# bartn8/vppstereo

Hardware: AMD Instinct MI355X
Metric: Mdisparities/s (HxWxD / s) VPP+rSGM at 540x960xD=192 (higher is better)
Workload: dtype u16

## Files before the change

vppstereo_amd/csrc/rsgm_kernels.hip:

```cpp
#include "vppx_internal.h"

#include <stdlib.h>

#define INVALID_DISP_COST 16u
#define INVALID_DISP (-10.0f)

typedef u32 u32x4 __attribute__((ext_vector_type(4)));
typedef u32 u32x2 __attribute__((ext_vector_type(2)));
typedef u16 u16x2 __attribute__((ext_vector_type(2)));

__device__ __forceinline__ u32 pk_min(u32 a, u32 b)
{
    u16x2 r = __builtin_elementwise_min(__builtin_bit_cast(u16x2, a), __builtin_bit_cast(u16x2, b));
    return __builtin_bit_cast(u32, r);
}
__device__ __forceinline__ u32 pk_adds(u32 a, u32 b)
{
    u16x2 r = __builtin_elementwise_add_sat(__builtin_bit_cast(u16x2, a), __builtin_bit_cast(u16x2, b));
    return __builtin_bit_cast(u32, r);
}
__device__ __forceinline__ u32 pk_sub(u32 a, u32 b)
{
    u16x2 r = __builtin_bit_cast(u16x2, a) - __builtin_bit_cast(u16x2, b);
    return __builtin_bit_cast(u32, r);
// ... 3724 lines not shown
    }
    return __builtin_amdgcn_fmed3f(fmaxf(fmaxf(lo[0], lo[1]), lo[2]), __builtin_amdgcn_fmed3f(md[0], md[1], md[2]),
                                   fminf(fminf(hi[0], hi[1]), hi[2]));
}
__global__ void __launch_bounds__(256) median3x3_kernel(const float *__restrict__ src, float *__restrict__ dst, int Hp, int Wp)
{
    const int x = blockIdx.x * blockDim.x + threadIdx.x;
    const int y = blockIdx.y;
    const int f = blockIdx.z;
    if (x >= Wp) return;
    const float *s = src + (size_t)f * Hp * Wp;
    float out;
    if (y == 0 || y == Hp - 1 || x == 0 || x == Wp - 1) {
        out = s[(size_t)y * Wp + x];
    } else {
        float v[9];
#pragma unroll
        for (int dy = -1; dy <= 1; dy++)
#pragma unroll
            for (int dx = -1; dx <= 1; dx++) v[(dy + 1) * 3 + dx + 1] = s[(size_t)(y + dy) * Wp + x + dx];
        out = median9(v);
    }
    dst[((size_t)f * Hp + y) * Wp + x] = out;
}

int rsgm_launch_median(vppx_ctx *ctx, int B, int Hp, int Wp, const float *src, float *dst)
{
    dim3 grid((Wp + 255) / 256, Hp, B);
    median3x3_kernel<<<grid, 256, 0, ctx->stream>>>(src, dst, Hp, Wp);
    VPPX_CHECK_LAUNCH();
    return 0;
}

__global__ void __launch_bounds__(256) median_interp_clip_kernel(ImgSet io, int B, int Hp, int Wp)
{
    extern __shared__ __attribute__((aligned(16))) float s_med[];
    const int nwords = (Wp + 63) / 64;
    unsigned long long *s_bits = (unsigned long long *)(s_med + ((Wp + 1) & ~1));
    const int y = blockIdx.x;
    const int set = blockIdx.y / B, f = blockIdx.y % B;
    const int lane = threadIdx.x & 63;
    const float *s = (const float *)(set == 0 ? io.src[0] : io.src[1]) + (size_t)f * Hp * Wp;
    float *dst = (float *)(set == 0 ? io.dst[0] : io.dst[1]) + ((size_t)f * Hp + y) * Wp;
    if (threadIdx.x == 0) s_bits[0] = 0ull, s_bits[nwords + 1] = 0ull;
    for (int xb = threadIdx.x & ~63; xb < Wp; xb += 256) {
        const int x = xb + lane;
        float out = 0.0f;
        if (x < Wp) {
            if (y == 0 || y == Hp - 1 || x == 0 || x == Wp - 1) {
                out = s[(size_t)y * Wp + x];
            } else {
                float v[9];
#pragma unroll
                for (int dy = -1; dy <= 1; dy++)
#pragma unroll
                    for (int dx = -1; dx <= 1; dx++) v[(dy + 1) * 3 + dx + 1] = s[(size_t)(y + dy) * Wp + x + dx];
                out = median9(v);
            }
            s_med[x] = out;
        }
        const unsigned long long bal = __builtin_amdgcn_ballot_w64(x < Wp && out > 0);
        if (lane == 0) s_bits[1 + (xb >> 6)] = bal;
    }
    __syncthreads();
    const float *row = s_med;
    const u32 *b32 = (const u32 *)s_bits;
    for (int x = threadIdx.x; x < Wp; x += 256) {
        float v = row[x];
        if (v <= 0) {
            const int sb = 64 + x - 13;
            const u32 w = __builtin_amdgcn_alignbit(b32[(sb >> 5) + 1], b32[sb >> 5], (u32)(sb & 31)) & 0x7FFFFFFu;
            const u32 wl = w & 0x1FFFu;
            int xl = -1, xr = -1;
            if (wl) {
                xl = x - 13 + (31 - __builtin_clz(wl));
                const int top = 27 - (x - xl);
                const u32 wr = (w >> 14) & ((1u << (top - 13)) - 1u);
                if (wr) xr = x + 1 + __builtin_ctz(wr);
            }
            if (xl >= 0 && xr >= 0) {
                const double n_left = (double)row[xl], n_right = (double)row[xr];
                if (fabs(n_left - n_right) < 3.0) {
                    const int xt = max(xl + 1, xr - 7);
                    const int n_leftx = xl - xt, n_rightx = xr - xt;
                    const double m = __ddiv_rn(n_right - n_left, (double)(n_rightx - n_leftx));
                    const double q = __dsub_rn(n_left, __dmul_rn(m, (double)n_leftx));
                    v = (float)__dadd_rn(__dmul_rn(m, (double)(x - xt)), q);
                }
            }
        }
        dst[x] = (v >= 0) ? v : 0.0f;
    }
}

int rsgm_launch_median_interp_clip(vppx_ctx *ctx, int B, int Hp, int Wp, const float *src_l, float *dst_l, const float *src_r,
                                   float *dst_r)
{
    ImgSet io;
    io.src[0] = src_l; io.dst[0] = dst_l; io.src[1] = src_r; io.dst[1] = dst_r; io.src[2] = nullptr; io.dst[2] = nullptr;
    const size_t lds = (size_t)((Wp + 1) & ~1) * sizeof(float) + (size_t)((Wp + 63) / 64 + 3) * sizeof(unsigned long long);
    median_interp_clip_kernel<<<dim3(Hp, 2 * B), 256, lds, ctx->stream>>>(io, B, Hp, Wp);
    VPPX_CHECK_LAUNCH();
    return 0;
}

__device__ __forceinline__ int uf_find(int *label, int i)
{
    int p = label[i];
    while (p != i) {
        i = p;
        p = label[i];
    }
    return i;
}
__device__ __forceinline__ int uf_find_halve(int *label, int i)
{
    int p = label[i];
    while (p != i) {
        const int gp = label[p];
        if (gp != p) atomicMin(&label[i], gp);
        i = p;
        p = gp;
    }
    return i;
}
__device__ __forceinline__ void uf_union(int *label, int a, int b)
{
    while (true) {
        a = uf_find_halve(label, a);
        b = uf_find_halve(label, b);
        if (a == b) return;
        if (a < b) { int t = a; a = b; b = t; }
        const int old = atomicMin(&label[a], b);
        if (old == a) return;
// ... 173 lines not shown
    }
    uf_union(lb, lb[ia], lb[ib]);
}

__global__ void __launch_bounds__(64) speckle_total_kernel(int *__restrict__ label, int *__restrict__ size, const int *__restrict__ roots,
                                                           const int *__restrict__ nroots, size_t npix_frame, int tiles_per_frame)
{
    const int tile = blockIdx.x;
    const size_t base = (size_t)(tile / tiles_per_frame) * npix_frame;
    int *lb = label + base;
    const int n = nroots[tile];
    const int *rl = roots + (size_t)tile * (SPK_TW * SPK_TH);
    for (int e = threadIdx.x; e < n; e += 64) {
        const int me = rl[e];
        const int sz = size[base + me];
        int c = me, p = lb[c];
        while (p != c) {
            const int gp = lb[p];
            if (gp != p) lb[c] = gp;
            c = gp;
            p = lb[c];
        }
        if (c != me) {
            lb[me] = c;
            atomicAdd(&size[base + c], sz);
        }
    }
}

template <int SEGMAX>
__global__ void __launch_bounds__(256) speckle_apply_rows_kernel(const u8 *__restrict__ fd8, const int *__restrict__ label,
                                                                  const int *__restrict__ size, const float *__restrict__ dl_pad,
                                                                  float *__restrict__ out, u8 *__restrict__ row_any, int H, int W, int Hp,
                                                                  int Wp, int pad_t, int pad_l, int new_val, int max_size, int subpixel)
{
    extern __shared__ __attribute__((aligned(16))) float sh_f[];
    __shared__ int s_l[4], s_r[4];
    float *val = sh_f, *res = sh_f + W;
    const int y = blockIdx.x, f = blockIdx.y;
    const int lane = threadIdx.x & 63, wv = threadIdx.x >> 6;
    const size_t base = (size_t)f * H * W, rowo = base + (size_t)y * W;
    const int *lb = label + base;
    const float *dlr = dl_pad + ((size_t)f * Hp + y + pad_t) * Wp + pad_l;
    float *g = out + rowo;
    for (int xb = threadIdx.x; xb < W; xb += 4 * 256) {
        int v[4], r1[4], r2[4];
        float sub[4];
#pragma unroll
        for (int u = 0; u < 4; u++) {
            const int x = min(xb + 256 * u, W - 1);
            v[u] = fd8[rowo + x];
            r1[u] = label[rowo + x];
            sub[u] = dlr[x];
        }
#pragma unroll
        for (int u = 0; u < 4; u++) r2[u] = lb[r1[u]];
#pragma unroll
        for (int u = 0; u < 4; u++) {
            int r = r1[u], pr = r2[u];
            while (pr != r) {
                r = pr;
                pr = lb[r];
            }
            r1[u] = r;
        }
        int sz[4];
#pragma unroll
        for (int u = 0; u < 4; u++) sz[u] = size[base + r1[u]];
#pragma unroll
        for (int u = 0; u < 4; u++) {
            const int x = xb + 256 * u;
            int vv = v[u];
            if (vv != new_val && sz[u] <= max_size) vv = new_val;
            float fv = (float)vv;
            if (subpixel && fv != 0.0f) fv = sub[u];
            if (x < W) val[x] = fv;
        }
// ... 25 lines not shown
    if (lane == 63) cr = 0x7FFFFFFF;
    for (int w = 0; w < wv; w++) cl = max(cl, s_l[w]);
    for (int w = wv + 1; w < 4; w++) cr = min(cr, s_r[w]);
    int xl[SEGMAX];
#pragma unroll
    for (int j = 0; j < SEGMAX; j++) {
        const int x = x0 + j;
        if (j < SEG && x < W && val[x] > 0) cl = x;
        xl[j] = cl;
    }
#pragma unroll
    for (int j = SEGMAX - 1; j >= 0; j--) {
        const int x = x0 + j;
        if (j >= SEG || x >= W) continue;
        float v = val[x];
        if (v > 0) {
            cr = x;
        } else {
            const bool hl = xl[j] >= 0, hr = cr < W;
            if (hl && hr) {
                const float a = val[xl[j]], b = val[cr];
                v = b < a ? b : a;
            } else if (hr) {
                v = val[cr];
            } else if (hl) {
                v = val[xl[j]];
            }
        }
        res[x] = v;
    }
    __syncthreads();
    for (int x = threadIdx.x; x < W; x += 256) g[x] = res[x];
}
__global__ void __launch_bounds__(256) interp_bg_edge_rows_kernel(float *__restrict__ dm, const u8 *__restrict__ row_any, int H, int W)
{
    __shared__ int s_first[4], s_last[4];
    const int f = blockIdx.x, lane = threadIdx.x & 63, wv = threadIdx.x >> 6;
    float *g = dm + (size_t)f * H * W;
    int first = 0x7FFFFFFF, last = -1;
    for (int v = threadIdx.x; v < H; v += 256)
        if (row_any[(size_t)f * H + v]) { first = min(first, v); last = max(last, v); }
#pragma unroll
    for (int off = 32; off >= 1; off >>= 1) {
        first = min(first, __shfl_xor(first, off));
        last = max(last, __shfl_xor(last, off));
    }
    if (lane == 0) s_first[wv] = first, s_last[wv] = last;
    __syncthreads();
    first = min(min(s_first[0], s_first[1]), min(s_first[2], s_first[3]));
    last = max(max(s_last[0], s_last[1]), max(s_last[2], s_last[3]));
    if (last < 0) return;
    for (size_t i = threadIdx.x; i < (size_t)first * W; i += 256) g[i] = g[(size_t)first * W + i % W];
    for (size_t i = (size_t)(last + 1) * W + threadIdx.x; i < (size_t)H * W; i += 256) g[i] = g[(size_t)last * W + i % W];
}

__global__ void __launch_bounds__(256) void_if_lost_kernel(float *__restrict__ out, size_t n, const unsigned *__restrict__ err_dev,
                                                           unsigned serial)
{
    if (__hip_atomic_load(err_dev, __ATOMIC_RELAXED, __HIP_MEMORY_SCOPE_AGENT) != serial) return;
    const float nan = __builtin_nanf("");
    for (size_t i = (size_t)blockIdx.x * 256 + threadIdx.x; i < n; i += (size_t)gridDim.x * 256) out[i] = nan;
}

int rsgm_launch_void_if_lost(vppx_ctx *ctx, float *out, size_t n, const unsigned *err_dev, unsigned serial)
{
    const unsigned nblk = (unsigned)((n + 256 * 16 - 1) / (256 * 16));
    void_if_lost_kernel<<<nblk < 1 ? 1 : nblk, 256, 0, ctx->stream>>>(out, n, err_dev, serial);
    VPPX_CHECK_LAUNCH();
    return 0;
}

int rsgm_launch_post(vppx_ctx *ctx, const RsgmGeom &g, const float *dl_pad, const float *dr_pad, int subpixel, float *out)
{
    const size_t n = (size_t)g.B * g.H * g.W, npf = (size_t)g.H * g.W;
    if (g.W > 8192) { vppx_set_error("frame width %d > 8192 is not supported by the post-processing kernels", g.W); return VPPX_E_UNSUPPORTED; }
    const int ntx = (g.W + SPK_TW - 1) / SPK_TW, nty = (g.H + SPK_TH - 1) / SPK_TH;
    const size_t ntiles = (size_t)ntx * nty * g.B;
    u8 *fd8, *row_any;
    int *label, *size, *roots, *nroots;
    int rc;
    if ((rc = ws_get(ctx, WS_FD8, n, &fd8))) return rc;
    if ((rc = ws_get(ctx, WS_LABEL, n, &label))) return rc;
    if ((rc = ws_get(ctx, WS_LCOUNT, n, &size))) return rc;
    if ((rc = ws_get(ctx, WS_SPK_ROOTS, ntiles * (SPK_TW * SPK_TH), &roots))) return rc;
    if ((rc = ws_get(ctx, WS_SPK_NROOTS, ntiles, &nroots))) return rc;
    if ((rc = ws_get(ctx, WS_ROW_ANY, (size_t)g.B * g.H, &row_any))) return rc;
    speckle_tile_kernel<<<dim3(ntx, nty, g.B), 256, 0, ctx->stream>>>(dl_pad, dr_pad, fd8, label, size, roots, nroots, g.H, g.W, g.Hp, g.Wp,
                                                                      g.pad_t, g.pad_l, 0, 10);
    VPPX_CHECK_LAUNCH();
    const int nby = (g.H - 1) / SPK_TH, nbx = (g.W - 1) / SPK_TW;
    const int nlinks = nby * g.W + nbx * g.H;
    if (nlinks > 0) {
        speckle_border_kernel<<<dim3((nlinks + 255) / 256, g.B), 256, 0, ctx->stream>>>(fd8, label, g.H, g.W, 0, 10);
        VPPX_CHECK_LAUNCH();
    }
    speckle_total_kernel<<<(unsigned)ntiles, 64, 0, ctx->stream>>>(label, size, roots, nroots, npf, ntx * nty);
    VPPX_CHECK_LAUNCH();
    const size_t lds = (size_t)g.W * 2 * sizeof(float);
    if (g.W <= 2048)
        speckle_apply_rows_kernel<8><<<dim3(g.H, g.B), 256, lds, ctx->stream>>>(fd8, label, size, dl_pad, out, row_any, g.H, g.W, g.Hp, g.Wp,
                                                                               g.pad_t, g.pad_l, 0, 200, subpixel);
    else
        speckle_apply_rows_kernel<32><<<dim3(g.H, g.B), 256, lds, ctx->stream>>>(fd8, label, size, dl_pad, out, row_any, g.H, g.W, g.Hp, g.Wp,
                                                                                g.pad_t, g.pad_l, 0, 200, subpixel);
    VPPX_CHECK_LAUNCH();
    interp_bg_edge_rows_kernel<<<g.B, 256, 0, ctx->stream>>>(out, row_any, g.H, g.W);
    VPPX_CHECK_LAUNCH();
    return 0;
}
```

vppstereo_amd/csrc/vpp_kernels.hip:

```cpp
#include "vppx_internal.h"

#include <math.h>
#include <string.h>
#include <mutex>
#include <stdlib.h>

#define LG 992
#define RLCAP 8

struct HintRec {
    int x;
    float g;
    u32 base;
    u32 flags;
};

__host__ __device__ inline int vpp_bits_words(int W) { return (W + 63) / 64 + 2; }

struct VppK {
    int B, H, W, C;
    int n, direction, uniform, discard, interp, use_dist, use_bil;
    int wsize_m1;
    float c, c_occ, dmin, dmax;
    const float2 *range;
// ... 2028 lines not shown
    const int x = blockIdx.x * blockDim.x + threadIdx.x;
    const int y = blockIdx.y, f = blockIdx.z;
    if (x >= W) return;
    const size_t fb = (size_t)f * H * W;
    auto unwarped = [&](int yy, int xx) -> float {
        const size_t row = fb + (size_t)yy * W;
        const int t = tmp[row + xx];
        return t < 0 ? 0.0f : omap[row + (t >> 1)];
    };
    float u = unwarped(y, x);
    if (u == 0.0f) {
        const float nl = x > 0 ? unwarped(y, x - 1) : unwarped(y, W - 1);
        const float nr = x < W - 1 ? unwarped(y, x + 1) : (y < H - 1 ? unwarped(y + 1, 0) : 0.0f);
        if (nl > 0 && nr > 0 && fabs(__dsub_rn((double)nl, (double)nr)) < 1.0) {
            const double m = __ddiv_rn(__dsub_rn((double)nr, (double)nl), 2.0);
            const double q = __dsub_rn((double)nl, __dmul_rn(m, -1.0));
            u = (float)__dadd_rn(__dmul_rn(m, 0.0), q);
        }
    }
    dmap_out[fb + (size_t)y * W + x] = u;
}

int occ_launch(vppx_ctx *ctx, int B, int H, int W, const float *hints, int rx, int ry, double l, double g,
               double th_conf, double th_filter, float *omap, u8 *conf_out, float *dmap_out)
{
    const size_t n = (size_t)B * H * W;
    const bool small = ctx->front_lds_budget < 12 * 1024;
    dim3 grid((W + 255) / 256, H, B), grid_t((W + (small ? 511 : 1023)) / (small ? 512 : 1024), H, B);
    int *tmp = nullptr;
    if (dmap_out) {
        int rc = ws_get(ctx, WS_OCC_TMP, n, &tmp);
        if (rc) return rc;
    }
    VPPX_HIP(hipMemsetAsync(omap, 0, n * sizeof(float), ctx->stream));
    if (W % 4 == 0 && ((size_t)hints & 15) == 0) {
        occ_warp4_kernel<<<dim3((W / 4 + 255) / 256, H, B), 256, 0, ctx->stream>>>((const float4 *)hints, (int *)omap, H, W);
        front_route_note(ctx, "occ_warp4");
    } else {
        occ_warp_kernel<<<grid, 256, 0, ctx->stream>>>(hints, (int *)omap, H, W);
        front_route_note(ctx, "occ_warp");
    }
    VPPX_CHECK_LAUNCH();
    rx /= 2, ry /= 2;
    const long long nwin = (2LL * rx + 1) * (2LL * ry + 2);
#define OCC_TEST(NJ) do { if (small) occ_test_kernel<NJ, 2><<<grid_t, 256, 0, ctx->stream>>>(hints, omap, conf_out, tmp, H, W, rx, ry, l, g, th_conf, th_filter); \
                          else occ_test_kernel<NJ, 4><<<grid_t, 256, 0, ctx->stream>>>(hints, omap, conf_out, tmp, H, W, rx, ry, l, g, th_conf, th_filter); \
                          front_route_note(ctx, "occ_test<%d,%d>", NJ, small ? 2 : 4); } while (0)
    if (nwin <= 64) OCC_TEST(1);
    else if (nwin <= 128) OCC_TEST(2);
    else if (nwin <= 192) OCC_TEST(3);
    else if (nwin <= 256) OCC_TEST(4);
    else OCC_TEST(0);
#undef OCC_TEST
    VPPX_CHECK_LAUNCH();
    if (dmap_out) {
        occ_dmap_kernel<<<grid, 256, 0, ctx->stream>>>(tmp, omap, dmap_out, H, W);
        VPPX_CHECK_LAUNCH();
        front_route_note(ctx, "occ_dmap");
    }
    return 0;
}
```

vppstereo_amd/csrc/vppx_api.hip:

```cpp
#include "vppx_internal.h"

#include <limits.h>
#include <math.h>
#include <stdarg.h>
#include <stdlib.h>
#include <string.h>

static thread_local char g_err[1024] = "";

void vppx_set_error(const char *fmt, ...)
{
    va_list ap;
    va_start(ap, fmt);
    vsnprintf(g_err, sizeof(g_err), fmt, ap);
    va_end(ap);
}

extern "C" const char *vppx_last_error(void) { return g_err; }

static void note_once(std::vector<std::string> &list, const char *name)
{
    for (const std::string &r : list)
        if (r == name) return;
    list.emplace_back(name);
// ... 835 lines not shown
    if (!ctx->stream_front) {
        VPPX_HIP(hipStreamCreateWithFlags(&ctx->stream_front, hipStreamNonBlocking));
        VPPX_HIP(hipEventCreateWithFlags(&ctx->ev_agg_done, hipEventDisableTiming));
        VPPX_HIP(hipEventCreateWithFlags(&ctx->ev_front_done, hipEventDisableTiming));
        VPPX_HIP(hipEventCreateWithFlags(&ctx->ev_inputs_auto, hipEventDisableTiming));
    }
    if (!ctx->have_agg_done) {
        VPPX_HIP(hipEventRecord(ctx->ev_agg_done, ctx->stream));
        ctx->have_agg_done = true;
        VPPX_HIP(hipStreamWaitEvent(ctx->stream_front, ctx->ev_agg_done, 0));
        if (ctx->inputs_ev) VPPX_HIP(hipStreamWaitEvent(ctx->stream_front, (hipEvent_t)ctx->inputs_ev, 0));
    } else {
        VPPX_HIP(hipStreamWaitEvent(ctx->stream_front, ctx->ev_agg_done, 0));
        if (ctx->inputs_ev) {
            VPPX_HIP(hipStreamWaitEvent(ctx->stream_front, (hipEvent_t)ctx->inputs_ev, 0));
        } else {
            VPPX_HIP(hipEventRecord(ctx->ev_inputs_auto, ctx->stream));
            VPPX_HIP(hipStreamWaitEvent(ctx->stream_front, ctx->ev_inputs_auto, 0));
        }
    }
    ctx->inputs_ev = nullptr;
    ctx->main_saved = ctx->stream;
    ctx->stream = ctx->stream_front;
    ctx->front_active = true;
    return 0;
}
static int front_end(vppx_ctx *ctx)
{
    if (!ctx->front_active) return 0;
    hipStream_t front = ctx->stream;
    ctx->stream = ctx->main_saved;
    ctx->front_active = false;
    VPPX_HIP(hipEventRecord(ctx->ev_front_done, front));
    if (ctx->xbuf_last && !ctx->xbuf_cleared && ctx->xbuf_last == ctx->ws[WS_VSTATE].p) {
        VPPX_HIP(hipMemsetAsync(ctx->xbuf_last, 0, ctx->xbuf_last_bytes, ctx->stream));
        ctx->xbuf_cleared = true;
    }
    if (ctx->occ_done_recorded) {
        bool any = false;
        for (int i = 0; i < ctx->n_pipe_copy; i++) any = any || ctx->pipe_copy[i].early;
        if (any) VPPX_HIP(hipStreamWaitEvent(ctx->stream, ctx->ev_occ_done, 0));
        for (int i = 0; i < ctx->n_pipe_copy; i++)
            if (ctx->pipe_copy[i].early)
                VPPX_HIP(hipMemcpyAsync(ctx->pipe_copy[i].dst, ctx->pipe_copy[i].src, ctx->pipe_copy[i].bytes, hipMemcpyDeviceToDevice, ctx->stream));
    }
    VPPX_HIP(hipStreamWaitEvent(ctx->stream, ctx->ev_front_done, 0));
    for (int i = 0; i < ctx->n_pipe_copy; i++)
        if (!(ctx->occ_done_recorded && ctx->pipe_copy[i].early))
            VPPX_HIP(hipMemcpyAsync(ctx->pipe_copy[i].dst, ctx->pipe_copy[i].src, ctx->pipe_copy[i].bytes, hipMemcpyDeviceToDevice, ctx->stream));
    ctx->n_pipe_copy = 0;
    ctx->occ_done_recorded = false;
    if (ctx->pipe_call && ctx->pipe_early) {
        VPPX_HIP(hipEventRecord(ctx->ev_agg_done, ctx->stream));
        ctx->have_agg_done = true;
    }
    return 0;
}
struct FrontGuard {
    vppx_ctx *ctx;
    ~FrontGuard()
    {
        if (ctx->front_active) {
            ctx->stream = ctx->main_saved;
            ctx->front_active = false;
        }
        ctx->pipe_call = false;
        ctx->n_pipe_copy = 0;
        ctx->occ_done_recorded = false;
    }
};

static int rsgm_core(vppx_ctx *ctx, const VppxRsgmParams &p, const RsgmGeom &g, const u8 *left, const u8 *left_vpp,
                     const u8 *right_vpp, float *disp_out, const float *hints = nullptr, const float *validhints = nullptr)
{
    int rc;
    const size_t npp = (size_t)g.B * g.Hp * g.Wp;
    const size_t ncell = npp * g.D;
    u8 *gl;
    u32 *cl, *cr_raw;
    const bool alt = ctx->pipe_call && (ctx->pipe_parity & 1);
    if (ctx->pipe_call) ctx->pipe_parity ^= 1;
    {
// ... 36 lines not shown
    }
    stage_mark(ctx, ST_AGGREGATE);
    ctx->last_B = g.B; ctx->last_Hp = g.Hp; ctx->last_Wp = g.Wp; ctx->last_D = g.D; ctx->last_rp = p; ctx->have_last = true;
    ctx->last_guided = hints && validhints;

    float *dl0, *dl1, *dr0, *dr1;
    if ((rc = ws_get(ctx, WS_DISP_L0, npp, &dl0))) return rc;
    if ((rc = ws_get(ctx, WS_DISP_L1, npp, &dl1))) return rc;
    if ((rc = ws_get(ctx, WS_DISP_R0, npp, &dr0))) return rc;
    if ((rc = ws_get(ctx, WS_DISP_R1, npp, &dr1))) return rc;
    const u32 fu = uniq_factor(p.uniqueness);
    if (ctx->wsum_route)
        rc = rsgm_launch_wsum(ctx, g.B, g.Hp, g.Wp, g.D, gl, cl, cr, lut_d, p.p1, vols[1], vols[2], vols[3], dl0, dr0, fu);
    else
        rc = rsgm_launch_sum_wta_lr(ctx, g.B, g.Hp, g.Wp, g.D, vols, nvol, elem_bytes, dl0, dr0, fu, 1,
                                    (hints && validhints) ? 0 : 24 + maxp2);
    if (rc < 0) return rc;
    if (rc == 0) {
        stage_mark(ctx, ST_SUM_WTA);
        ctx->last_sum_nvol = nvol; ctx->last_sum_D = g.D; ctx->last_sum_B = g.B;
    } else {
        ctx->last_sum_nvol = 0;
        u16 *S;
        if ((rc = ws_get(ctx, WS_S, ncell, &S))) return rc;
        if ((rc = rsgm_launch_sum_wta(ctx, g.B, g.Hp, g.Wp, g.D, vols[0], elem_bytes, nullptr, S, dl0, fu, 1))) return rc;
        stage_mark(ctx, ST_SUM_WTA);
        if ((rc = rsgm_launch_wta_right_t(ctx, g.B, g.Hp, g.Wp, g.D, S, dr0, fu))) return rc;
        stage_mark(ctx, ST_WTA_RIGHT);
    }
    if ((rc = rsgm_launch_median_interp_clip(ctx, g.B, g.Hp, g.Wp, dl0, dl1, dr0, dr1))) return rc;
    stage_mark(ctx, ST_MEDIAN_INTERP);
    { float *t = dl0; dl0 = dl1; dl1 = t; t = dr0; dr0 = dr1; dr1 = t; }

    const size_t np = (size_t)g.B * g.H * g.W;
    if ((rc = rsgm_launch_post(ctx, g, dl0, dr0, p.subpixel, disp_out))) return rc;
    if (ctx->last_vert == 3 && ctx->ws[WS_V3ERR].p &&
        (rc = rsgm_launch_void_if_lost(ctx, disp_out, np, (const unsigned *)ctx->ws[WS_V3ERR].p, ctx->v3.serial))) return rc;
    stage_mark(ctx, ST_POST);
    return 0;
}

static int check_frames(int B, int H, int W, int C)
{
    if (B <= 0 || H <= 0 || W <= 0) { vppx_set_error("bad shape B=%d H=%d W=%d", B, H, W); return VPPX_E_INVALID_ARG; }
    if (C != 1 && C != 3) { vppx_set_error("channels must be 1 or 3 (got %d)", C); return VPPX_E_INVALID_ARG; }
    if (H < 5 || W < 5) { vppx_set_error("frame too small (%dx%d)", H, W); return VPPX_E_INVALID_ARG; }
    return 0;
}

static int guided_frames_per_part(const vppx_ctx *ctx, int H, int W, int C, int dmax)
{
    RsgmGeom g1;
    make_geom(1, H, W, C, dmax, g1);
    const unsigned long long per = (unsigned long long)g1.Hp * g1.Wp * g1.D * 16ull;
    const unsigned long long n = ctx->knobs.guided_part_bytes / per;
    return n < 1 ? 1 : (n > (unsigned long long)INT_MAX ? INT_MAX : (int)n);
}

extern "C" int vppx_rsgm_dev(vppx_ctx *ctx, const VppxRsgmParams *p, int B, int H, int W, int C, const uint8_t *left,
                             const uint8_t *left_vpp, const uint8_t *right_vpp, const float *hints,
                             const float *validhints, float *disp_out)
{
    int rc;
    VPPX_ENTER(ctx);
    routes_reset(ctx);
    if ((rc = lockstep_check(ctx))) return rc;
    if (!p || !left || !left_vpp || !right_vpp || !disp_out) { vppx_set_error("vppx_rsgm: NULL argument"); return VPPX_E_INVALID_ARG; }
    if ((rc = check_frames(B, H, W, C))) return rc;
    if ((rc = check_rsgm_params(*p))) return rc;
    if ((hints == nullptr) != (validhints == nullptr)) { hints = nullptr; validhints = nullptr; }
// ... 269 lines not shown
    const u8 *const left = c.left, *const right = c.right, *g_occ = c.g_occ;
    const float *const g = c.g;
    u8 *l_vpp = c.l_vpp, *r_vpp = c.r_vpp, *const conf_out = c.conf_out;
    const size_t nb = (size_t)B * H * W * C, np = (size_t)B * H * W;
    const bool piped = pipeline_applies(ctx);
    u8 *l_user = l_vpp, *r_user = r_vpp, *conf_user = conf_out;
    if ((piped || !l_vpp) && (rc = ws_get(ctx, WS_VPP_L, nb, &l_vpp))) return rc;
    if ((piped || !r_vpp) && (rc = ws_get(ctx, WS_VPP_R, nb, &r_vpp))) return rc;
    float *omap = nullptr;
    u8 *conf = conf_out;
    if (op) {
        if ((rc = ws_get(ctx, WS_OCC_OMAP, np, &omap))) return rc;
        if ((piped || !conf_out) && (rc = ws_get(ctx, WS_OCC_OUT, np, &conf))) return rc;
    }
    FrontGuard guard{ctx};
    ctx->n_pipe_copy = 0;
    if (piped) {
        ctx->pipe_call = true;
        if ((rc = front_begin(ctx))) return rc;
        ctx->occ_done_recorded = false;
        if (op && conf_user) ctx->pipe_copy[ctx->n_pipe_copy++] = {conf_user, conf, np, true};
        if (l_user) ctx->pipe_copy[ctx->n_pipe_copy++] = {l_user, l_vpp, nb, false};
        if (r_user) ctx->pipe_copy[ctx->n_pipe_copy++] = {r_user, r_vpp, nb, false};
    }
    {
        const int nvol_prev = (ctx->last_sum_nvol && ctx->last_sum_D == rp->dmax && ctx->last_sum_B == B) ? ctx->last_sum_nvol
                                                                                                          : (B >= VPPX_FUSED_MIN_FRAMES ? 4 : 8);
        const size_t sum_lds = rsgm_sum_lds_bytes(ctx, rp->dmax, nvol_prev), cu_lds = 160 * 1024;
        const size_t left_over = cu_lds > sum_lds + 512 ? cu_lds - sum_lds - 512 : 2048;
        const bool sum_fills_cu = rp->dmax == 256 && nvol_prev == 4 && ctx->knobs.sum_trap == 2 && !ctx->knobs.sum_general;
        ctx->front_lds_budget = (piped && !sum_fills_cu && left_over < 64 * 1024 && left_over >= 6 * 1024) ? left_over : 64 * 1024;
    }
    stage_begin(ctx);
    if (op) {
        if ((rc = occ_launch(ctx, B, H, W, g, op->rx, op->ry, op->l, op->g, op->th_conf, op->th_filter, omap, conf))) return rc;
        stage_mark(ctx, ST_OCC);
        g_occ = conf;
        if (piped && conf_user) {
            if (!ctx->ev_occ_done) VPPX_HIP(hipEventCreateWithFlags(&ctx->ev_occ_done, hipEventDisableTiming));
            VPPX_HIP(hipEventRecord(ctx->ev_occ_done, ctx->stream));
            ctx->occ_done_recorded = true;
        }
    }
    VPPX_HIP(hipMemcpyAsync(l_vpp, left, nb, hipMemcpyDeviceToDevice, ctx->stream));
    VPPX_HIP(hipMemcpyAsync(r_vpp, right, nb, hipMemcpyDeviceToDevice, ctx->stream));
    VppGeom vg = {B, H, W, C};
    const float *filled_g = nullptr;
    if (vp->use_bilateral_patch) {
        float *fg;
        if ((rc = ws_get(ctx, WS_FILLED_G, (size_t)B * H * W, &fg))) return rc;
        if ((rc = vpp_launch_bilateral_fill(ctx, *vp, vg, left, g, fg))) return rc;
        filled_g = fg;
    }
    if ((rc = vpp_launch(ctx, *vp, vg, l_vpp, r_vpp, g, g_occ, filled_g, nullptr, nullptr, right))) return rc;
    if (ctx->draws_dst && vp->method == VPPX_METHOD_RND)
        VPPX_HIP(hipMemcpy2DAsync(ctx->draws_dst, 8, ctx->ws[WS_FRAME_TOT].p, 16, 8, (size_t)B, hipMemcpyDeviceToDevice, ctx->stream));
    RsgmGeom rg;
    make_geom(B, H, W, C, rp->dmax, rg);
    return rsgm_core(ctx, *rp, rg, left, l_vpp, r_vpp, c.disp_out, c.validhints ? g : nullptr, c.validhints);
}

static int vpp_rsgm_entry(vppx_ctx *ctx, const HotCall &c);
static int scaled_call(vppx_ctx *ctx, const HotCall &c);
static int eval_call(vppx_ctx *ctx, const HotCall &c);
static int sampled_call(vppx_ctx *ctx, const HotCall &c);

static HotCall hot_call(HotCall::Layer layer, const VppxOccParams *op, const VppxVppParams *vp, const VppxRsgmParams *rp, int B, int H, int W,
                        int C, const uint8_t *left, const uint8_t *right)
{
    HotCall c;
    c.layer = layer;
    c.op = op;
    if (vp) c.vp = *vp;
    c.vp_null = !vp;
    c.rp = rp;
    c.B = B; c.H = H; c.W = W; c.C = C;
    c.left = left; c.right = right;
    return c;
// ... 1340 lines not shown
```

vppstereo_amd/csrc/vppx_internal.h:

```cpp
#pragma once
#include <hip/hip_runtime.h>
#include <stdint.h>
#include <stdio.h>
#include <string>
#include <vector>

#include "../../include/vppx.h"

typedef uint8_t u8;
typedef uint16_t u16;
typedef uint32_t u32;
typedef uint64_t u64;

void vppx_set_error(const char *fmt, ...);

#define VPPX_HIP(call)                                                                              \
    do {                                                                                            \
        hipError_t e_ = (call);                                                                     \
        if (e_ != hipSuccess) {                                                                     \
            vppx_set_error("%s failed: %s (%s:%d)", #call, hipGetErrorString(e_), __FILE__, __LINE__); \
            return VPPX_E_HIP;                                                                      \
        }                                                                                           \
    } while (0)

// ... 390 lines not shown
int rsgm_vert3_frames_per_round(const vppx_ctx *ctx, int Wp, int D);
bool rsgm_vert3_wide(const vppx_ctx *ctx, int B, int Wp, int D);
size_t rsgm_vert3_xbuf_bytes(int B, int Wp, int D);
void rsgm_vert3_plan(const vppx_ctx *ctx, int B, int Wp, int D, int *whole_frames, bool *rest_underfilled);
int rsgm_launch_vert3_range(vppx_ctx *ctx, hipStream_t stream, int B_total, int f0, int nB, int Hp, int Wp, int D, const u8 *gray,
                            const u32 *cl, const u32 *cr, const u16 *p2lut, int p1, u8 *sv, u32 *xbuf, unsigned *err, unsigned *err_dev,
                            bool next_to_we);
int rsgm_launch_vert3(vppx_ctx *ctx, hipStream_t stream, int B, int Hp, int Wp, int D, const u8 *gray, const u32 *cl,
                      const u32 *cr, const u16 *p2lut, int p1, u8 *sv, u32 *xbuf, unsigned *err, unsigned *err_dev);
int rsgm_launch_void_if_lost(vppx_ctx *ctx, float *out, size_t n, const unsigned *err_dev, unsigned serial);
bool rsgm_vert_supported(int D, int maxp2);
size_t rsgm_vert_state_bytes(int B, int Wp, int D);
size_t rsgm_vert_min_elems(int B, int Wp);
int rsgm_launch_vert(vppx_ctx *ctx, hipStream_t stream, int B, int Hp, int Wp, int D, const u8 *gray, const u32 *cl,
                     const u32 *cr, const u16 *p2lut, int p1, u8 *sv, u8 *gst, u16 *gmin);
int rsgm_launch_sum_wta(vppx_ctx *ctx, int B, int Hp, int Wp, int D, const void *paths, int elem_bytes, u16 *S,
                        u16 *ST, float *disp_l, u32 factor_uniq, int do_subpixel);
int rsgm_launch_wta_right_t(vppx_ctx *ctx, int B, int Hp, int Wp, int D, const u16 *ST, float *disp, u32 factor_uniq);
int rsgm_paths_elem_bytes(int D, int maxp2);
size_t rsgm_sum_lds_bytes(const vppx_ctx *ctx, int D, int nvol);
bool rsgm_wsum_default(int B, int Hp, int Wp, int D, int maxp2, int nsimd);
bool rsgm_wsum_eligible(const vppx_ctx *ctx, int B, int Hp, int Wp, int D, int maxp2, int nsimd);
int rsgm_device_simds(vppx_ctx *ctx);
int rsgm_launch_wsum(vppx_ctx *ctx, int B, int Hp, int Wp, int D, const u8 *gray, const u32 *cl, const u32 *cr, const u16 *p2lut, int p1,
                     const void *vol_e, const void *vol_n3, const void *vol_s3, float *disp_l, float *disp_r, u32 fu);
int rsgm_launch_sum_wta_lr(vppx_ctx *ctx, int B, int Hp, int Wp, int D, const void *const *vols, int nvol, int elem_bytes,
                           float *disp_l, float *disp_r, u32 factor_uniq, int do_subpixel, int max_path_value);
int rsgm_launch_wta_left(vppx_ctx *ctx, int B, int Hp, int Wp, int D, const u16 *S, float *disp, u32 factor_uniq);
int rsgm_launch_subpixel(vppx_ctx *ctx, int B, int Hp, int Wp, int D, const u16 *S, float *disp);
int rsgm_launch_wta_right(vppx_ctx *ctx, int B, int Hp, int Wp, int D, const u16 *S, float *disp, u32 factor_uniq);
int rsgm_launch_median(vppx_ctx *ctx, int B, int Hp, int Wp, const float *src, float *dst);
int rsgm_launch_median_interp_clip(vppx_ctx *ctx, int B, int Hp, int Wp, const float *src_l, float *dst_l, const float *src_r,
                                   float *dst_r);
int rsgm_launch_post(vppx_ctx *ctx, const RsgmGeom &g, const float *dl_pad, const float *dr_pad, int subpixel, float *out);

struct VppGeom {
    int B, H, W, C;
};
int vpp_launch(vppx_ctx *ctx, const VppxVppParams &p, const VppGeom &g, u8 *l, u8 *r, const float *gmap,
               const u8 *occ, const float *filled_g, int64_t *n_hints_dev, const u32 *seeds_dev, const u8 *r_orig = nullptr);
int vpp_launch_bilateral_fill(vppx_ctx *ctx, const VppxVppParams &p, const VppGeom &g, const u8 *left, const float *gmap,
                              float *filled_out);
int vpp_launch_rand_stream(vppx_ctx *ctx, u32 seed, u64 offset, int64_t n, int32_t *out_dev);
u64 vpp_draws_upper_bound(const VppxVppParams &p, const VppGeom &g);

int handoff_psmnet_cost_volume(vppx_ctx *ctx, const void *fl, const void *fr, const float *hints, const float *valid, int B, int C,
                               int H4, int W4, int H, int W, int maxdisp, void *cost, int dtype);
int handoff_raft_corr_modulate(vppx_ctx *ctx, void *corr, const float *hints, const float *valid, int B, int H4, int W2, int W3, int H,
                               int W, int dtype);
int handoff_kitti_decode(vppx_ctx *ctx, const uint16_t *png, size_t n, float *disp, u8 *valid);
int handoff_pfm_decode(vppx_ctx *ctx, const u8 *raw, int H, int W, int channels, int little, float *out);
int handoff_subsample_hints(vppx_ctx *ctx, const float *hints, const float *valid, int B, int H, int W, int H4, int W4, float **hs,
                            float **vs, int raft);
int corr_pyramid(vppx_ctx *ctx, void *corr, const float *hints, const float *valid, int B, int H4, int W2, int W3, int H, int W,
                 int levels, void *pyr, int dtype);
int corr_lookup(vppx_ctx *ctx, const void *corr, const void *pyr, const float *coords_x, int64_t coords_frame_stride, int B, int H4,
                int W2, int W3, int levels, int radius, float *out, int dtype);
int corr_fused(vppx_ctx *ctx, const void *fmap2, const void *fmap3, const float *hints, const float *valid, int B, int D, int H4,
               int W2, int W3, int H, int W, int levels, void *corr, void *pyr, int dtype);
static inline int64_t corr_pyramid_offsets(int64_t N, int W3, int levels, int64_t *off)
{
    int64_t cells = 0;
    if (off) off[0] = 0;
    for (int i = 1; i < levels; i++) {
        if (off) off[i] = cells;
        cells += N * (int64_t)(W3 >> i);
    }
// ... 93 lines not shown
```

Baseline: 435,200.

## Batch memcpys/memsets into one copy kernel, stage median rows in LDS, fold void check

Several hipMemcpyAsync and hipMemsetAsync calls on the stream become a single custom copy/zero kernel that takes up to four jobs per launch, which cuts the number of stream operations. The left/right image copies move ahead of the occlusion stage. The median+interp kernel gains an LDS-staged path that computes per-column vertical min/med/max once from float4 loads, so each 3x3 median needs fewer global reads. The separate void-if-lost launch is folded into the post kernels through an error-flag check. The trade-off is extra LDS per block and a hand-written copy kernel standing in for the runtime's DMA path.

```diff
diff --git a/vppstereo_amd/csrc/rsgm_kernels.hip b/vppstereo_amd/csrc/rsgm_kernels.hip
--- a/vppstereo_amd/csrc/rsgm_kernels.hip
+++ b/vppstereo_amd/csrc/rsgm_kernels.hip
@@ -3780,9 +3780,11 @@
     return 0;
 }
 
+template <bool STAGED>
 __global__ void __launch_bounds__(256) median_interp_clip_kernel(ImgSet io, int B, int Hp, int Wp)
 {
-    extern __shared__ __attribute__((aligned(16))) float s_med[];
+    extern __shared__ __attribute__((aligned(16))) float s_all[];
+    float *s_med = s_all + (STAGED ? 3 * Wp : 0);
     const int nwords = (Wp + 63) / 64;
     unsigned long long *s_bits = (unsigned long long *)(s_med + ((Wp + 1) & ~1));
     const int y = blockIdx.x;
@@ -3791,12 +3793,43 @@
     const float *s = (const float *)(set == 0 ? io.src[0] : io.src[1]) + (size_t)f * Hp * Wp;
     float *dst = (float *)(set == 0 ? io.dst[0] : io.dst[1]) + ((size_t)f * Hp + y) * Wp;
     if (threadIdx.x == 0) s_bits[0] = 0ull, s_bits[nwords + 1] = 0ull;
+    const bool edge_row = y == 0 || y == Hp - 1;
+    const float *s_lo = s_all, *s_md = s_all + Wp, *s_hi = s_all + 2 * Wp;
+    if (STAGED) {
+        if (!edge_row) {
+            for (int x4 = threadIdx.x * 4; x4 < Wp; x4 += 4 * 256) {
+                const float4 a = *(const float4 *)(s + (size_t)(y - 1) * Wp + x4), b = *(const float4 *)(s + (size_t)y * Wp + x4),
+                             d = *(const float4 *)(s + (size_t)(y + 1) * Wp + x4);
+                float4 lo, md, hi;
+                lo.x = fminf(fminf(a.x, b.x), d.x); md.x = __builtin_amdgcn_fmed3f(a.x, b.x, d.x); hi.x = fmaxf(fmaxf(a.x, b.x), d.x);
+                lo.y = fminf(fminf(a.y, b.y), d.y); md.y = __builtin_amdgcn_fmed3f(a.y, b.y, d.y); hi.y = fmaxf(fmaxf(a.y, b.y), d.y);
+                lo.z = fminf(fminf(a.z, b.z), d.z); md.z = __builtin_amdgcn_fmed3f(a.z, b.z, d.z); hi.z = fmaxf(fmaxf(a.z, b.z), d.z);
+                lo.w = fminf(fminf(a.w, b.w), d.w); md.w = __builtin_amdgcn_fmed3f(a.w, b.w, d.w); hi.w = fmaxf(fmaxf(a.w, b.w), d.w);
+                *(float4 *)(s_all + x4) = lo;
+                *(float4 *)(s_all + Wp + x4) = md;
+                *(float4 *)(s_all + 2 * Wp + x4) = hi;
+                if (x4 == 0) s_med[0] = b.x;
+                if (x4 + 4 == Wp) s_med[Wp - 1] = b.w;
+            }
+        }
+        __syncthreads();
+    }
     for (int xb = threadIdx.x & ~63; xb < Wp; xb += 256) {
         const int x = xb + lane;
         float out = 0.0f;
         if (x < Wp) {
-            if (y == 0 || y == Hp - 1 || x == 0 || x == Wp - 1) {
+            if (STAGED && !edge_row) {
+                if (x == 0 || x == Wp - 1) {
+                    out = s_med[x];
+                } else {
+                    out = __builtin_amdgcn_fmed3f(fmaxf(fmaxf(s_lo[x - 1], s_lo[x]), s_lo[x + 1]),
+                                                  __builtin_amdgcn_fmed3f(s_md[x - 1], s_md[x], s_md[x + 1]),
+                                                  fminf(fminf(s_hi[x - 1], s_hi[x]), s_hi[x + 1]));
+                    s_med[x] = out;
+                }
+            } else if (edge_row || x == 0 || x == Wp - 1) {
                 out = s[(size_t)y * Wp + x];
+                s_med[x] = out;
             } else {
                 float v[9];
 #pragma unroll
@@ -3804,8 +3837,8 @@
 #pragma unroll
                     for (int dx = -1; dx <= 1; dx++) v[(dy + 1) * 3 + dx + 1] = s[(size_t)(y + dy) * Wp + x + dx];
                 out = median9(v);
-            }
-            s_med[x] = out;
+                s_med[x] = out;
+            }
         }
         const unsigned long long bal = __builtin_amdgcn_ballot_w64(x < Wp && out > 0);
         if (lane == 0) s_bits[1 + (xb >> 6)] = bal;
@@ -3847,7 +3880,11 @@
     ImgSet io;
     io.src[0] = src_l; io.dst[0] = dst_l; io.src[1] = src_r; io.dst[1] = dst_r; io.src[2] = nullptr; io.dst[2] = nullptr;
     const size_t lds = (size_t)((Wp + 1) & ~1) * sizeof(float) + (size_t)((Wp + 63) / 64 + 3) * sizeof(unsigned long long);
-    median_interp_clip_kernel<<<dim3(Hp, 2 * B), 256, lds, ctx->stream>>>(io, B, Hp, Wp);
+    const size_t lds_staged = lds + (size_t)3 * Wp * sizeof(float);
+    if (Wp % 4 == 0 && lds_staged <= 64 * 1024 && (((uintptr_t)src_l | (uintptr_t)src_r) & 15) == 0)
+        median_interp_clip_kernel<true><<<dim3(Hp, 2 * B), 256, lds_staged, ctx->stream>>>(io, B, Hp, Wp);
+    else
+        median_interp_clip_kernel<false><<<dim3(Hp, 2 * B), 256, lds, ctx->stream>>>(io, B, Hp, Wp);
     VPPX_CHECK_LAUNCH();
     return 0;
 }
@@ -4087,7 +4124,8 @@
 __global__ void __launch_bounds__(256) speckle_apply_rows_kernel(const u8 *__restrict__ fd8, const int *__restrict__ label,
                                                                   const int *__restrict__ size, const float *__restrict__ dl_pad,
                                                                   float *__restrict__ out, u8 *__restrict__ row_any, int H, int W, int Hp,
-                                                                  int Wp, int pad_t, int pad_l, int new_val, int max_size, int subpixel)
+                                                                  int Wp, int pad_t, int pad_l, int new_val, int max_size, int subpixel,
+                                                                  const unsigned *__restrict__ err_dev, unsigned serial)
 {
     extern __shared__ __attribute__((aligned(16))) float sh_f[];
     __shared__ int s_l[4], s_r[4];
@@ -4098,6 +4136,11 @@
     const int *lb = label + base;
     const float *dlr = dl_pad + ((size_t)f * Hp + y + pad_t) * Wp + pad_l;
     float *g = out + rowo;
+    if (err_dev && __hip_atomic_load(err_dev, __ATOMIC_RELAXED, __HIP_MEMORY_SCOPE_AGENT) == serial) {
+        const float nan = __builtin_nanf("");
+        for (int x = threadIdx.x; x < W; x += 256) g[x] = nan;
+        return;
+    }
     for (int xb = threadIdx.x; xb < W; xb += 4 * 256) {
         int v[4], r1[4], r2[4];
         float sub[4];
@@ -4189,9 +4232,11 @@
     __syncthreads();
     for (int x = threadIdx.x; x < W; x += 256) g[x] = res[x];
 }
-__global__ void __launch_bounds__(256) interp_bg_edge_rows_kernel(float *__restrict__ dm, const u8 *__restrict__ row_any, int H, int W)
+__global__ void __launch_bounds__(256) interp_bg_edge_rows_kernel(float *__restrict__ dm, const u8 *__restrict__ row_any, int H, int W,
+                                                                  const unsigned *__restrict__ err_dev, unsigned serial)
 {
     __shared__ int s_first[4], s_last[4];
+    if (err_dev && __hip_atomic_load(err_dev, __ATOMIC_RELAXED, __HIP_MEMORY_SCOPE_AGENT) == serial) return;
     const int f = blockIdx.x, lane = threadIdx.x & 63, wv = threadIdx.x >> 6;
     float *g = dm + (size_t)f * H * W;
     int first = 0x7FFFFFFF, last = -1;
@@ -4227,7 +4272,8 @@
     return 0;
 }
 
-int rsgm_launch_post(vppx_ctx *ctx, const RsgmGeom &g, const float *dl_pad, const float *dr_pad, int subpixel, float *out)
+int rsgm_launch_post(vppx_ctx *ctx, const RsgmGeom &g, const float *dl_pad, const float *dr_pad, int subpixel, float *out,
+                     const unsigned *err_dev, unsigned serial)
 {
     const size_t n = (size_t)g.B * g.H * g.W, npf = (size_t)g.H * g.W;
     if (g.W > 8192) { vppx_set_error("frame width %d > 8192 is not supported by the post-processing kernels", g.W); return VPPX_E_UNSUPPORTED; }
@@ -4256,12 +4302,93 @@
     const size_t lds = (size_t)g.W * 2 * sizeof(float);
     if (g.W <= 2048)
         speckle_apply_rows_kernel<8><<<dim3(g.H, g.B), 256, lds, ctx->stream>>>(fd8, label, size, dl_pad, out, row_any, g.H, g.W, g.Hp, g.Wp,
-                                                                               g.pad_t, g.pad_l, 0, 200, subpixel);
+                                                                               g.pad_t, g.pad_l, 0, 200, subpixel, err_dev, serial);
     else
         speckle_apply_rows_kernel<32><<<dim3(g.H, g.B), 256, lds, ctx->stream>>>(fd8, label, size, dl_pad, out, row_any, g.H, g.W, g.Hp, g.Wp,
-                                                                                g.pad_t, g.pad_l, 0, 200, subpixel);
+                                                                                g.pad_t, g.pad_l, 0, 200, subpixel, err_dev, serial);
     VPPX_CHECK_LAUNCH();
-    interp_bg_edge_rows_kernel<<<g.B, 256, 0, ctx->stream>>>(out, row_any, g.H, g.W);
+    interp_bg_edge_rows_kernel<<<g.B, 256, 0, ctx->stream>>>(out, row_any, g.H, g.W, err_dev, serial);
     VPPX_CHECK_LAUNCH();
     return 0;
 }
+
+struct HandoffArgs {
+    u8 *dst[VPPX_HANDOFF_MAX];
+    const u8 *src[VPPX_HANDOFF_MAX];
+    size_t bytes[VPPX_HANDOFF_MAX];
+    unsigned blk0[VPPX_HANDOFF_MAX];
+    int n;
+};
+constexpr int HO_UNROLL = 4;
+struct __attribute__((packed, aligned(1))) HoUnit { u32 w[4]; };
+template <int NT>
+__global__ void __launch_bounds__(NT) handoff_kernel(HandoffArgs a)
+{
+    u8 *dst = a.dst[0];
+    const u8 *src = a.src[0];
+    size_t bytes = a.bytes[0];
+    unsigned b0 = 0;
+#pragma unroll
+    for (int j = 1; j < VPPX_HANDOFF_MAX; j++)
+        if (j < a.n && blockIdx.x >= a.blk0[j]) { dst = a.dst[j]; src = a.src[j]; bytes = a.bytes[j]; b0 = a.blk0[j]; }
+    const unsigned lb = blockIdx.x - b0;
+    size_t head = (size_t)(-(uintptr_t)dst & 15);
+    head = head < bytes ? head : bytes;
+    const size_t units = (bytes - head) >> 4, tail0 = head + (units << 4);
+    if (lb == 0) {
+        if (threadIdx.x < head) dst[threadIdx.x] = src ? src[threadIdx.x] : (u8)0;
+        const size_t t = tail0 + threadIdx.x;
+        if (t < bytes) dst[t] = src ? src[t] : (u8)0;
+    }
+    uint4 *d = (uint4 *)(dst + head);
+    const size_t u0 = (size_t)lb * (NT * HO_UNROLL) + threadIdx.x;
+    uint4 v[HO_UNROLL];
+    if (!src) {
+#pragma unroll
+        for (int k = 0; k < HO_UNROLL; k++) v[k] = make_uint4(0, 0, 0, 0);
+    } else if ((((uintptr_t)src + head) & 15) == 0) {
+        const uint4 *s = (const uint4 *)(src + head);
+#pragma unroll
+        for (int k = 0; k < HO_UNROLL; k++) {
+            const size_t u = u0 + NT * k;
+            if (u < units) v[k] = s[u];
+        }
+    } else {
+        const HoUnit *s = (const HoUnit *)(src + head);
+#pragma unroll
+        for (int k = 0; k < HO_UNROLL; k++) {
+            const size_t u = u0 + NT * k;
+            if (u < units) {
+                const HoUnit t = s[u];
+                v[k] = make_uint4(t.w[0], t.w[1], t.w[2], t.w[3]);
+            }
+        }
+    }
+#pragma unroll
+    for (int k = 0; k < HO_UNROLL; k++) {
+        const size_t u = u0 + NT * k;
+        if (u < units) d[u] = v[k];
+    }
+}
+
+int rsgm_launch_handoff(vppx_ctx *ctx, const HandoffJob *jobs, int n, bool single_wave)
+{
+    const size_t per_block = (size_t)(single_wave ? 64 : 256) * HO_UNROLL;
+    HandoffArgs a = {};
+    unsigned nblk = 0;
+    for (int i = 0; i < n; i++) {
+        if (!jobs[i].bytes) continue;
+        if (a.n == VPPX_HANDOFF_MAX) { vppx_set_error("hand-off launch: more than %d jobs", VPPX_HANDOFF_MAX); return VPPX_E_INVALID_ARG; }
+        const size_t blocks = (jobs[i].bytes / 16 + per_block - 1) / per_block;
+        if (blocks + 1 > 0x7FFFFFFFull - nblk) { vppx_set_error("hand-off launch: %zu bytes are too many", jobs[i].bytes); return VPPX_E_UNSUPPORTED; }
+        a.dst[a.n] = (u8 *)jobs[i].dst; a.src[a.n] = (const u8 *)jobs[i].src; a.bytes[a.n] = jobs[i].bytes;
+        a.blk0[a.n] = nblk;
+        nblk += blocks < 1 ? 1u : (unsigned)blocks;
+        a.n++;
+    }
+    if (!a.n) return 0;
+    if (single_wave) handoff_kernel<64><<<nblk, 64, 0, ctx->stream>>>(a);
+    else handoff_kernel<256><<<nblk, 256, 0, ctx->stream>>>(a);
+    VPPX_CHECK_LAUNCH();
+    return 0;
+}
diff --git a/vppstereo_amd/csrc/vpp_kernels.hip b/vppstereo_amd/csrc/vpp_kernels.hip
--- a/vppstereo_amd/csrc/vpp_kernels.hip
+++ b/vppstereo_amd/csrc/vpp_kernels.hip
@@ -2084,7 +2084,11 @@
         int rc = ws_get(ctx, WS_OCC_TMP, n, &tmp);
         if (rc) return rc;
     }
-    VPPX_HIP(hipMemsetAsync(omap, 0, n * sizeof(float), ctx->stream));
+    {
+        const HandoffJob zero = {omap, nullptr, n * sizeof(float)};
+        const int rc = rsgm_launch_handoff(ctx, &zero, 1, true);
+        if (rc) return rc;
+    }
     if (W % 4 == 0 && ((size_t)hints & 15) == 0) {
         occ_warp4_kernel<<<dim3((W / 4 + 255) / 256, H, B), 256, 0, ctx->stream>>>((const float4 *)hints, (int *)omap, H, W);
         front_route_note(ctx, "occ_warp4");
diff --git a/vppstereo_amd/csrc/vppx_api.hip b/vppstereo_amd/csrc/vppx_api.hip
--- a/vppstereo_amd/csrc/vppx_api.hip
+++ b/vppstereo_amd/csrc/vppx_api.hip
@@ -891,8 +891,11 @@
     ctx->stream = ctx->main_saved;
     ctx->front_active = false;
     VPPX_HIP(hipEventRecord(ctx->ev_front_done, front));
+    int rc;
+    HandoffJob jobs[VPPX_HANDOFF_MAX];
+    int nj = 0;
     if (ctx->xbuf_last && !ctx->xbuf_cleared && ctx->xbuf_last == ctx->ws[WS_VSTATE].p) {
-        VPPX_HIP(hipMemsetAsync(ctx->xbuf_last, 0, ctx->xbuf_last_bytes, ctx->stream));
+        jobs[nj++] = {ctx->xbuf_last, nullptr, ctx->xbuf_last_bytes};
         ctx->xbuf_cleared = true;
     }
     if (ctx->occ_done_recorded) {
@@ -900,13 +903,15 @@
         for (int i = 0; i < ctx->n_pipe_copy; i++) any = any || ctx->pipe_copy[i].early;
         if (any) VPPX_HIP(hipStreamWaitEvent(ctx->stream, ctx->ev_occ_done, 0));
         for (int i = 0; i < ctx->n_pipe_copy; i++)
-            if (ctx->pipe_copy[i].early)
-                VPPX_HIP(hipMemcpyAsync(ctx->pipe_copy[i].dst, ctx->pipe_copy[i].src, ctx->pipe_copy[i].bytes, hipMemcpyDeviceToDevice, ctx->stream));
-    }
+            if (ctx->pipe_copy[i].early) jobs[nj++] = {ctx->pipe_copy[i].dst, ctx->pipe_copy[i].src, ctx->pipe_copy[i].bytes};
+    }
+    if ((rc = rsgm_launch_handoff(ctx, jobs, nj))) return rc;
+    nj = 0;
     VPPX_HIP(hipStreamWaitEvent(ctx->stream, ctx->ev_front_done, 0));
     for (int i = 0; i < ctx->n_pipe_copy; i++)
         if (!(ctx->occ_done_recorded && ctx->pipe_copy[i].early))
-            VPPX_HIP(hipMemcpyAsync(ctx->pipe_copy[i].dst, ctx->pipe_copy[i].src, ctx->pipe_copy[i].bytes, hipMemcpyDeviceToDevice, ctx->stream));
+            jobs[nj++] = {ctx->pipe_copy[i].dst, ctx->pipe_copy[i].src, ctx->pipe_copy[i].bytes};
+    if ((rc = rsgm_launch_handoff(ctx, jobs, nj))) return rc;
     ctx->n_pipe_copy = 0;
     ctx->occ_done_recorded = false;
     if (ctx->pipe_call && ctx->pipe_early) {
@@ -1009,10 +1014,9 @@
     stage_mark(ctx, ST_MEDIAN_INTERP);
     { float *t = dl0; dl0 = dl1; dl1 = t; t = dr0; dr0 = dr1; dr1 = t; }
 
-    const size_t np = (size_t)g.B * g.H * g.W;
-    if ((rc = rsgm_launch_post(ctx, g, dl0, dr0, p.subpixel, disp_out))) return rc;
-    if (ctx->last_vert == 3 && ctx->ws[WS_V3ERR].p &&
-        (rc = rsgm_launch_void_if_lost(ctx, disp_out, np, (const unsigned *)ctx->ws[WS_V3ERR].p, ctx->v3.serial))) return rc;
+    const bool voidable = ctx->last_vert == 3 && ctx->ws[WS_V3ERR].p;
+    if ((rc = rsgm_launch_post(ctx, g, dl0, dr0, p.subpixel, disp_out, voidable ? (const unsigned *)ctx->ws[WS_V3ERR].p : nullptr,
+                               ctx->v3.serial))) return rc;
     stage_mark(ctx, ST_POST);
     return 0;
 }
@@ -1348,6 +1352,10 @@
         ctx->front_lds_budget = (piped && !sum_fills_cu && left_over < 64 * 1024 && left_over >= 6 * 1024) ? left_over : 64 * 1024;
     }
     stage_begin(ctx);
+    {
+        const HandoffJob pair[2] = {{l_vpp, left, nb}, {r_vpp, right, nb}};
+        if ((rc = rsgm_launch_handoff(ctx, pair, 2, true))) return rc;
+    }
     if (op) {
         if ((rc = occ_launch(ctx, B, H, W, g, op->rx, op->ry, op->l, op->g, op->th_conf, op->th_filter, omap, conf))) return rc;
         stage_mark(ctx, ST_OCC);
@@ -1358,8 +1366,6 @@
             ctx->occ_done_recorded = true;
         }
     }
-    VPPX_HIP(hipMemcpyAsync(l_vpp, left, nb, hipMemcpyDeviceToDevice, ctx->stream));
-    VPPX_HIP(hipMemcpyAsync(r_vpp, right, nb, hipMemcpyDeviceToDevice, ctx->stream));
     VppGeom vg = {B, H, W, C};
     const float *filled_g = nullptr;
     if (vp->use_bilateral_patch) {
diff --git a/vppstereo_amd/csrc/vppx_internal.h b/vppstereo_amd/csrc/vppx_internal.h
--- a/vppstereo_amd/csrc/vppx_internal.h
+++ b/vppstereo_amd/csrc/vppx_internal.h
@@ -446,7 +446,11 @@
 int rsgm_launch_median(vppx_ctx *ctx, int B, int Hp, int Wp, const float *src, float *dst);
 int rsgm_launch_median_interp_clip(vppx_ctx *ctx, int B, int Hp, int Wp, const float *src_l, float *dst_l, const float *src_r,
                                    float *dst_r);
-int rsgm_launch_post(vppx_ctx *ctx, const RsgmGeom &g, const float *dl_pad, const float *dr_pad, int subpixel, float *out);
+int rsgm_launch_post(vppx_ctx *ctx, const RsgmGeom &g, const float *dl_pad, const float *dr_pad, int subpixel, float *out,
+                     const unsigned *err_dev = nullptr, unsigned serial = 0);
+#define VPPX_HANDOFF_MAX 4
+struct HandoffJob { void *dst; const void *src; size_t bytes; };
+int rsgm_launch_handoff(vppx_ctx *ctx, const HandoffJob *jobs, int n, bool single_wave = false);
 
 struct VppGeom {
     int B, H, W, C;
```

Measured after the change: 437,500 (median of 6 runs). About the same (+0.5%).
